# SensorsINI/v2e

Measured on NVIDIA H100. Metric: Mevents/s, higher is better.
Workload: dtype fp16 tensor-core convs (fp32 accumulate) + f64 pixel state

## Files before the change

### include/v2e_b200.h

```cpp
#ifndef V2E_B200_H
#define V2E_B200_H

#include <stdint.h>

#ifdef __cplusplus
extern "C" {
#endif

typedef enum V2eStatus {
    V2E_OK = 0,
    V2E_E_INVALID = -1,
    V2E_E_CUDA = -2,
    V2E_E_CAPACITY = -3,
    V2E_E_ITER_CAP = -4,
    V2E_E_STATE = -5,
    V2E_E_UNSUPPORTED = -6,
    V2E_E_FALLBACK = -7
} V2eStatus;

typedef enum V2eFrameDtype { V2E_U8 = 0, V2E_F32 = 1, V2E_F64 = 2 } V2eFrameDtype;

const char *v2e_last_error(void);
int v2e_version(void);
int v2e_abi_info(int *version, int *emu_cfg_size, int *frame_info_size, int *unet_weights_size);
// ... 97 lines not shown
int v2e_emu_read_counts(V2eEmu *h, int32_t *max_n, uint32_t *counts_host, int counts_cap,
                        void *stream);
int v2e_emu_phase_shot(V2eEmu *h, const void *frame_dev, int frame_dtype, double t_frame,
                       double t_previous, const float *shot_rand_dev, uint64_t capacity,
                       void *stream);
int v2e_emu_phase_emit(V2eEmu *h, double t_frame, double t_previous, float *events_out_dev,
                       uint64_t capacity, void *stream);

int v2e_emu_profile(V2eEmu *h, int enable);
int v2e_emu_profile_read4(V2eEmu *h, float *ms_sum4, int *launches4, void *stream);

int v2e_emu_state_is_f64(V2eEmu *h);
void *v2e_emu_state_ptr(V2eEmu *h, int which);

int v2e_emu_draw_noise(V2eEmu *h, uint32_t frame_index, float *leak_randn, float *shot_u01, float *pr_randn,
                       void *stream);


int v2e_conv2d_lrelu_sm100(const void *x1_dev, int C1, const void *x2_dev, int C2,
                           const void *wgt_dev, const float *bias_dev, int Cout_pad, int KH, int KW,
                           int N, int H, int W, void *out_dev, int out_cstride, int out_mode,
                           int co_real, float slope, void *stream);

int v2e_conv2d_lrelu_sm100_strip(const void *x1_dev, int C1, const void *x2_dev, int C2,
                                 const void *wgt_row_dev, const float *bias_dev, int Cout_pad, int KH,
                                 int KW, int N, int H, int W, void *out_dev, int out_cstride,
                                 int out_mode, int co_real, float slope, void *stream);
int v2e_conv_strip_pick_kc(int C1, int C2, int Cout_pad, int KH, int KW, int W);

int v2e_conv2d_up2_lrelu_sm100(const void *x_low_dev, int C, const void *wgt_fold_dev, const void *wgt_plain_dev,
                               const float *bias_dev, int Cout_pad, int N, int H_out, int W_out, void *out_dev,
                               int out_cstride, float slope, void *stream);
int v2e_conv_up2_fold_weights(const float *w_host, int cout, int cin, int Cout_pad, int C_pad, void *out_host);
int v2e_conv_up2_supported_c(int C, int Cout_pad, int W_out);

typedef struct V2eUNetWeights {
    const float *w[23];
    const float *b[23];
} V2eUNetWeights;

typedef struct V2eSlomo V2eSlomo;

int v2e_slomo_create(int H, int W, int max_batch, const V2eUNetWeights *flow,
                     const V2eUNetWeights *interp, V2eSlomo **out);
int v2e_slomo_destroy(V2eSlomo *h);
int v2e_slomo_set_pairs(V2eSlomo *h, const uint8_t *frames_u8_dev, int B, void *stream);
// ... 62 lines not shown
```

### v2e_b200/_lib.py

```python
import ctypes
import os

from . import build as _build

_LIB = None


class V2eEmuCfg(ctypes.Structure):
    _fields_ = [
        ("width", ctypes.c_int32), ("height", ctypes.c_int32),
        ("per_pixel_thres", ctypes.c_int32), ("hdr", ctypes.c_int32),
        ("pos_thres_nominal", ctypes.c_double), ("neg_thres_nominal", ctypes.c_double),
        ("cutoff_hz", ctypes.c_double), ("leak_rate_hz", ctypes.c_double),
        ("leak_jitter_fraction", ctypes.c_double), ("refractory_period_s", ctypes.c_double),
        ("shot_noise_rate_hz", ctypes.c_double), ("shot_inten_factor", ctypes.c_double),
        ("rng_mode", ctypes.c_int32), ("iter_cap", ctypes.c_int32),
        ("seed", ctypes.c_uint64),
        ("csdvs", ctypes.c_int32), ("max_frames_per_step", ctypes.c_int32),
        ("cs_tau_p_s", ctypes.c_double), ("cs_tau_h_s", ctypes.c_double),
        ("scidvs", ctypes.c_int32), ("photoreceptor_noise", ctypes.c_int32),
        ("rng_pixel_offset", ctypes.c_uint32), ("full_frame_px", ctypes.c_uint32),
        ("own_row0", ctypes.c_int32), ("own_rows", ctypes.c_int32),
        ("cs_halo_rows", ctypes.c_int32), ("reserved1", ctypes.c_int32),
    ]
# ... 39 lines not shown
    "v2e_emu_set_linlog_lut": (_i, [_vp, _vp, _vp]),
    "v2e_emu_set_fields": (_i, [_vp, _vp, _vp, _vp]),
    "v2e_emu_first_frame": (_i, [_vp, _vp, _i, _d, _d, _vp]),
    "v2e_emu_step": (_i, [_vp, _vp, _i, _i, _vp, _d, _vp, _vp, _vp, _u64, _u64, _i, _i, _vp]),
    "v2e_emu_collect": (_i, [_vp, ctypes.POINTER(V2eFrameInfo), _i, ctypes.POINTER(_i),
                             ctypes.POINTER(_u64), _vp]),
    "v2e_emu_phase_count": (_i, [_vp, _vp, _i, _d, _d, _vp, _vp, _i, _u64, _u64, _vp]),
    "v2e_emu_phase_update": (_i, [_vp, _vp, _i, _d, _d, _vp, _vp, _u64, _u64, _vp]),
    "v2e_emu_max_n_dev": (_vp, [_vp]),
    "v2e_emu_cs_begin": (_i, [_vp, _vp, _i, _d, _d, _u64, _u64, ctypes.POINTER(_i), _vp]),
    "v2e_emu_cs_pack": (_i, [_vp, _vp]),
    "v2e_emu_cs_unpack_from": (_i, [_vp, _vp, _vp, _vp]),
    "v2e_emu_cs_send_dev": (_vp, [_vp]),
    "v2e_emu_cs_chunk": (_i, [_vp, _i, _i, _vp]),
    "v2e_emu_cs_max_dev": (_vp, [_vp]),
    "v2e_emu_cs_advance": (_i, [_vp, _i, _i, _vp]),
    "v2e_emu_cs_update": (_i, [_vp, _vp, _i, _vp, _vp, _vp]),
    "v2e_emu_phase_filter": (_i, [_vp, _d, _d, _u64, _i, _vp]),
    "v2e_emu_read_counts": (_i, [_vp, ctypes.POINTER(ctypes.c_int32), _vp, _i, _vp]),
    "v2e_emu_phase_shot": (_i, [_vp, _vp, _i, _d, _d, _vp, _u64, _vp]),
    "v2e_emu_phase_emit": (_i, [_vp, _d, _d, _vp, _u64, _vp]),
    "v2e_conv2d_lrelu_sm100": (_i, [_vp, _i, _vp, _i, _vp, _vp, _i, _i, _i, _i, _i, _i, _vp, _i, _i, _i,
                                    ctypes.c_float, _vp]),
    "v2e_conv2d_lrelu_sm100_strip": (_i, [_vp, _i, _vp, _i, _vp, _vp, _i, _i, _i, _i, _i, _i, _vp, _i, _i, _i,
                                          ctypes.c_float, _vp]),
    "v2e_conv_strip_pick_kc": (_i, [_i, _i, _i, _i, _i, _i]),
    "v2e_conv2d_up2_lrelu_sm100": (_i, [_vp, _i, _vp, _vp, _vp, _i, _i, _i, _i, _vp, _i, ctypes.c_float, _vp]),
    "v2e_conv_up2_fold_weights": (_i, [_vp, _i, _i, _i, _i, _vp]),
    "v2e_conv_up2_supported_c": (_i, [_i, _i, _i]),
    "v2e_slomo_create": (_i, [_i, _i, _i, _vp, _vp, ctypes.POINTER(_vp)]),
    "v2e_slomo_destroy": (_i, [_vp]),
    "v2e_slomo_set_pairs": (_i, [_vp, _vp, _i, _vp]),
    "v2e_slomo_max_flow": (_i, [_vp, ctypes.POINTER(ctypes.c_float), _vp]),
    "v2e_slomo_interp": (_i, [_vp, _d, _vp, _vp, _vp]),
    "v2e_slomo_set_option": (_i, [_vp, _i, _i]),
    "v2e_slomo_check_finite": (_i, [_vp, ctypes.POINTER(_i), _vp]),
    "v2e_slomo_profile": (_i, [_vp, _i]),
    "v2e_slomo_profile_read": (_i, [_vp, ctypes.POINTER(ctypes.c_float), ctypes.POINTER(_i),
                                    ctypes.POINTER(ctypes.c_double), _vp]),
    "v2e_slomo_profile_read_layers": (_i, [_vp, ctypes.POINTER(ctypes.c_float), ctypes.POINTER(_i),
                                           ctypes.POINTER(ctypes.c_double), ctypes.POINTER(ctypes.c_float),
                                           ctypes.POINTER(_i), ctypes.POINTER(ctypes.c_double), _vp]),
    "v2e_slomo_flow_ptr": (_vp, [_vp]),
    "v2e_slomo_intrp_ptr": (_vp, [_vp]),
    "v2e_slomo_buffer_ptr": (_vp, [_vp, _i, _i]),
    "v2e_slomo_layer_kernel": (_i, [_vp, _i, _i]),
# ... 75 lines not shown
```

### v2e_b200/csrc/conv_tc.cu

```cuda
#include <cuda.h>
#include <cuda_fp16.h>
#include <cuda_runtime.h>
#include <stdint.h>
#include <stdio.h>
#include <string.h>
#include <vector>
#include <stdlib.h>

#include "../../include/v2e_b200.h"
#include "common.cuh"
#include "tc_common.cuh"

namespace {

constexpr int kTileH = 8, kTileW = 16, kBM = kTileH * kTileW;
constexpr int kStages = 4;
constexpr int kConvThreads = 288;
constexpr int kProducerWarp = 8;
constexpr int kConsumerWarps = 8;

struct ConvParams {
    int N, H, W;
    int C1, C2;
    int KH, KW;
    int KC;
    int BN;
    int stages;
    int co_fast;
    int tiles_x, tiles_y;
    int out_cstride;
    int out_mode;
    int co_real;
    float slope;
    const float *bias;
    void *out;
};

__device__ __forceinline__ uint8_t *align1024(uint8_t *p) { return (uint8_t *)(((uintptr_t)p + 1023) & ~(uintptr_t)1023); }

__device__ __forceinline__ float lrelu(float x, float slope) { return x > 0.f ? x : x * slope; }

template <int BN>
__device__ __forceinline__ void epilogue_row(const float (&d)[BN / 2], int i, bool inb, size_t pix, int lane,
                                             const float *bias, float slope, int out_mode, void *out, int cstride,
                                             int co0, __half2 (&h)[BN / 8]) {
#pragma unroll
    for (int j = 0; j < BN / 8; j++) {
        const int c = 8 * j + 2 * (lane & 3);
        const float x0 = lrelu(d[4 * j + 2 * i] + __ldg(bias + c), slope);
        const float x1 = lrelu(d[4 * j + 2 * i + 1] + __ldg(bias + c + 1), slope);
        h[j] = __floats2half2_rn(x0, x1);
        if (inb) {
// ... 69 lines not shown
            const uint32_t base = (uint32_t)stage * stage16;
            wgmma_fence();
            for (int j = 0; j < ksteps; j++)
                wgmma_f16<BN>(acc, desc_add(d0, base + (uint32_t)g * half16 + 2u * j), desc_add(d0, base + a16 + 2u * j),
                              (uint32_t)((it | j) != 0));
            wgmma_commit();
            wgmma_wait<1>();
            if (prev >= 0) { __syncwarp(); if (lane == 0) mbar_arrive(&empty_bar[prev]); }
            prev = stage;
            if (++stage == p.stages) { stage = 0; phase ^= 1; }
        }
        wgmma_wait<0>();
        wgmma_fence_regs(acc);
        __half2 hv[BN / 8];
#pragma unroll
        for (int i = 0; i < 2; i++) {
            const int m = 64 * g + 16 * (warp & 3) + (lane >> 2) + 8 * i;
            const int py = y0 + m / kTileW, px = x0 + m % kTileW;
            const bool inb = py < p.H && px < p.W;
            const size_t pix = ((size_t)n * p.H + py) * p.W + px;
            epilogue_row<BN>(acc, i, inb, pix, lane, p.bias + n0, p.slope, p.out_mode, p.out, p.out_cstride, n0, hv);
        }
    }
}


constexpr int kRowTile = 128;

struct StripParams {
    int N, H, W;
    int C1, C2;
    int KH, KW;
    int KC, BN;
    int tiles_x, seg_h, n_seg, n_items;
    int nslot;
    void *pool_out;
    int pool_cstride;
    int n_split, cout_pad;
    int slab_bytes;
    int w_bytes;
    int out_cstride, out_mode, co_real;
    float slope;
    const float *bias;
    void *out;
};
constexpr int kMaxSlot = 12;
// ... 379 lines not shown
extern int v2e_set_error(int code, const char *fmt, const char *detail);

typedef CUresult (*EncodeTiledFn)(CUtensorMap *, CUtensorMapDataType, cuuint32_t, void *, const cuuint64_t *,
                                  const cuuint64_t *, const cuuint32_t *, const cuuint32_t *,
                                  CUtensorMapInterleave, CUtensorMapSwizzle, CUtensorMapL2promotion,
                                  CUtensorMapFloatOOBfill);

static EncodeTiledFn encode_fn() {
    static EncodeTiledFn fn = nullptr;
    if (!fn) {
        void *p = nullptr;
        cudaDriverEntryPointQueryResult q;
        if (cudaGetDriverEntryPoint("cuTensorMapEncodeTiled", &p, cudaEnableDefault, &q) == cudaSuccess &&
            q == cudaDriverEntryPointSuccess)
            fn = (EncodeTiledFn)p;
    }
    return fn;
}

static CUtensorMapSwizzle swizzle_for(int kc) {
    return kc == 64 ? CU_TENSOR_MAP_SWIZZLE_128B : (kc == 32 ? CU_TENSOR_MAP_SWIZZLE_64B : CU_TENSOR_MAP_SWIZZLE_32B);
}

int v2e_make_act_tmap(CUtensorMap *tm, const void *ptr, int N, int H, int W, int C, int KC) {
    EncodeTiledFn fn = encode_fn();
    if (!fn) return v2e_set_error(V2E_E_CUDA, "cuTensorMapEncodeTiled unavailable%s", "");
    cuuint64_t dims[4] = {(cuuint64_t)C, (cuuint64_t)W, (cuuint64_t)H, (cuuint64_t)N};
    cuuint64_t strides[3] = {(cuuint64_t)C * 2, (cuuint64_t)W * C * 2, (cuuint64_t)H * W * C * 2};
    cuuint32_t box[4] = {(cuuint32_t)KC, (cuuint32_t)kTileW, (cuuint32_t)kTileH, 1};
    cuuint32_t es[4] = {1, 1, 1, 1};
    CUresult r = fn(tm, CU_TENSOR_MAP_DATA_TYPE_FLOAT16, 4, (void *)ptr, dims, strides, box, es,
                    CU_TENSOR_MAP_INTERLEAVE_NONE, swizzle_for(KC), CU_TENSOR_MAP_L2_PROMOTION_L2_256B,
                    CU_TENSOR_MAP_FLOAT_OOB_FILL_NONE);
    if (r != CUDA_SUCCESS) {
        snprintf(g_conv_err, sizeof(g_conv_err), "activation map N=%d H=%d W=%d C=%d KC=%d CUresult=%d", N, H, W, C, KC, (int)r);
        return v2e_set_error(V2E_E_CUDA, "cuTensorMapEncodeTiled failed: %s", g_conv_err);
    }
    return V2E_OK;
}

int v2e_make_wgt_tmap(CUtensorMap *tm, const void *ptr, int Cout_pad, int Ktot, int KC, int BN) {
    EncodeTiledFn fn = encode_fn();
    if (!fn) return v2e_set_error(V2E_E_CUDA, "cuTensorMapEncodeTiled unavailable%s", "");
    cuuint64_t dims[2] = {(cuuint64_t)Ktot, (cuuint64_t)Cout_pad};
    cuuint64_t strides[1] = {(cuuint64_t)Ktot * 2};
    cuuint32_t box[2] = {(cuuint32_t)KC, (cuuint32_t)BN};
    cuuint32_t es[2] = {1, 1};
    CUresult r = fn(tm, CU_TENSOR_MAP_DATA_TYPE_FLOAT16, 2, (void *)ptr, dims, strides, box, es,
                    CU_TENSOR_MAP_INTERLEAVE_NONE, swizzle_for(KC), CU_TENSOR_MAP_L2_PROMOTION_L2_256B,
                    CU_TENSOR_MAP_FLOAT_OOB_FILL_NONE);
    if (r != CUDA_SUCCESS) {
        snprintf(g_conv_err, sizeof(g_conv_err), "weight map Cout=%d K=%d KC=%d BN=%d CUresult=%d", Cout_pad, Ktot, KC, BN, (int)r);
        return v2e_set_error(V2E_E_CUDA, "cuTensorMapEncodeTiled failed: %s", g_conv_err);
    }
    return V2E_OK;
}

int v2e_conv_pick_kc(int C1, int C2) {
    int g = C2 ? (C1 < C2 ? C1 : C2) : C1;
    return g % 64 == 0 ? 64 : (g % 32 == 0 ? 32 : 16);
}
int v2e_conv_pick_bn(int Cout_pad) { return Cout_pad >= 128 ? 128 : Cout_pad; }

struct V2eConvLaunch {
    CUtensorMap tmA, tmA2, tmB;
    ConvParams p;
    dim3 grid;
    size_t smem;
};

int v2e_conv_prepare(V2eConvLaunch *L, const void *x1, int C1, const void *x2, int C2, const void *wgt,
                     const float *bias, int Cout_pad, int KH, int KW, int N, int H, int W, void *out,
                     int out_cstride, int out_mode, int co_real, float slope) {
    if (C1 % 16 || C2 % 16 || !(Cout_pad == 16 || Cout_pad == 32 || Cout_pad == 64 || (Cout_pad > 0 && Cout_pad % 128 == 0)))
        return v2e_set_error(V2E_E_INVALID, "conv: channel counts must be padded to 16 (Cout to 16/32/64/128k)%s", "");
    memset(L, 0, sizeof(*L));
    ConvParams &p = L->p;
    p.N = N; p.H = H; p.W = W; p.C1 = C1; p.C2 = C2; p.KH = KH; p.KW = KW;
    p.KC = v2e_conv_pick_kc(C1, C2);
    p.BN = v2e_conv_pick_bn(Cout_pad);
    p.stages = kStages;
    p.tiles_x = (W + kTileW - 1) / kTileW;
    p.tiles_y = (H + kTileH - 1) / kTileH;
    p.out_cstride = out_cstride; p.out_mode = out_mode; p.co_real = co_real; p.slope = slope;
    p.bias = bias; p.out = out;
    int rc;
    if ((rc = v2e_make_act_tmap(&L->tmA, x1, N, H, W, C1, p.KC))) return rc;
    if (C2) { if ((rc = v2e_make_act_tmap(&L->tmA2, x2, N, H, W, C2, p.KC))) return rc; }
    else L->tmA2 = L->tmA;
    if ((rc = v2e_make_wgt_tmap(&L->tmB, wgt, Cout_pad, KH * KW * (C1 + C2), p.KC, p.BN))) return rc;
    {
        static int co_fast = -1;
        if (co_fast < 0) { const char *e = getenv("V2E_CONV_CO_FAST"); co_fast = e ? atoi(e) : 1; }
        const unsigned tiles = (unsigned)(p.tiles_x * p.tiles_y * N), cob = (unsigned)(Cout_pad / p.BN);
        p.co_fast = (co_fast && cob > 1 && tiles <= 65535u) ? 1 : 0;
        L->grid = p.co_fast ? dim3(cob, tiles, 1) : dim3(tiles, cob, 1);
    }
    size_t stage = (size_t)kBM * p.KC * 2 + (((size_t)p.BN * p.KC * 2 + 1023) & ~(size_t)1023);
    L->smem = stage * p.stages + 1024;
    return V2E_OK;
}

template <int BN>
static cudaError_t conv_launch_bn(const V2eConvLaunch *L, cudaStream_t st) {
    static PerDeviceOnce attr_once;
    if (attr_once.first()) cudaFuncSetAttribute(conv_tc_kernel<BN>, cudaFuncAttributeMaxDynamicSharedMemorySize, 200 * 1024);
    conv_tc_kernel<BN><<<L->grid, kConvThreads, L->smem, st>>>(L->tmA, L->tmA2, L->tmB, L->p);
    return cudaGetLastError();
}

int v2e_conv_launch(const V2eConvLaunch *L, cudaStream_t st) {
    cudaError_t e;
    switch (L->p.BN) {
        case 16: e = conv_launch_bn<16>(L, st); break;
        case 32: e = conv_launch_bn<32>(L, st); break;
        case 64: e = conv_launch_bn<64>(L, st); break;
        case 128: e = conv_launch_bn<128>(L, st); break;
        default: return v2e_set_error(V2E_E_UNSUPPORTED, "conv_tc_kernel: unsupported tile width%s", "");
    }
    if (e != cudaSuccess) return v2e_set_error(V2E_E_CUDA, "conv_tc_kernel launch: %s", cudaGetErrorString(e));
    return V2E_OK;
}

size_t v2e_conv_launch_size(void) { return sizeof(V2eConvLaunch); }

extern "C" int v2e_conv2d_lrelu_sm100(const void *x1_dev, int C1, const void *x2_dev, int C2,
                                      const void *wgt_dev, const float *bias_dev, int Cout_pad, int KH, int KW,
                                      int N, int H, int W, void *out_dev, int out_cstride, int out_mode,
                                      int co_real, float slope, void *stream) {
    V2eConvLaunch L;
    int rc = v2e_conv_prepare(&L, x1_dev, C1, x2_dev, C2, wgt_dev, bias_dev, Cout_pad, KH, KW, N, H, W, out_dev,
                              out_cstride, out_mode, co_real, slope);
    if (rc) return rc;
    return v2e_conv_launch(&L, (cudaStream_t)stream);
}

struct V2eStripLaunch {
    CUtensorMap tmA, tmA2, tmB;
    StripParams p;
    int grid;
    size_t smem;
};

static int make_rowseg_tmap(CUtensorMap *tm, const void *ptr, int N, int H, int W, int C, int KC, int KW) {
    EncodeTiledFn fn = encode_fn();
    if (!fn) return v2e_set_error(V2E_E_CUDA, "cuTensorMapEncodeTiled unavailable%s", "");
    cuuint64_t dims[4] = {(cuuint64_t)C, (cuuint64_t)W, (cuuint64_t)H, (cuuint64_t)N};
    cuuint64_t strides[3] = {(cuuint64_t)C * 2, (cuuint64_t)W * C * 2, (cuuint64_t)H * W * C * 2};
    cuuint32_t box[4] = {(cuuint32_t)KC, (cuuint32_t)(kRowTile + KW - 1), 1, 1};
    cuuint32_t es[4] = {1, 1, 1, 1};
    CUresult r = fn(tm, CU_TENSOR_MAP_DATA_TYPE_FLOAT16, 4, (void *)ptr, dims, strides, box, es,
                    CU_TENSOR_MAP_INTERLEAVE_NONE, swizzle_for(KC), CU_TENSOR_MAP_L2_PROMOTION_L2_256B,
                    CU_TENSOR_MAP_FLOAT_OOB_FILL_NONE);
    if (r != CUDA_SUCCESS) return v2e_set_error(V2E_E_CUDA, "cuTensorMapEncodeTiled failed for a strip row map%s", "");
    return V2E_OK;
}

// ... 305 lines not shown
```

### v2e_b200/csrc/slomo.cu

```cuda
#include <cuda.h>
#include <cuda_fp16.h>
#include <cuda_runtime.h>
#include <math.h>
#include <stdint.h>
#include <stdio.h>
#include <string.h>
#include <stdlib.h>

#include <vector>

#include "../../include/v2e_b200.h"
#include "common.cuh"

struct V2eConvLaunch;
int v2e_conv_prepare(V2eConvLaunch *L, const void *x1, int C1, const void *x2, int C2, const void *wgt,
                     const float *bias, int Cout_pad, int KH, int KW, int N, int H, int W, void *out,
                     int out_cstride, int out_mode, int co_real, float slope);
int v2e_conv_launch(const V2eConvLaunch *L, cudaStream_t st);
size_t v2e_conv_launch_size(void);
struct V2eStripLaunch;
int v2e_strip_pick(int C1, int C2, int Cout_pad, int KH, int KW, int W, int *nslot_out);
size_t v2e_strip_launch_size(void);
int v2e_strip_pool_supported(int C1, int C2, int Cout_pad, int KH, int KW, int H, int W);
int v2e_strip_prepare(V2eStripLaunch *L, const void *x1, int C1, const void *x2, int C2, const void *wgt_row,
                      const float *bias, int Cout_pad, int KH, int KW, int N, int H, int W, void *out,
                      int out_cstride, int out_mode, int co_real, float slope, int n_sms, void *pool_out,
                      int pool_cstride);
int v2e_strip_launch(const V2eStripLaunch *L, cudaStream_t st);
struct V2eUpLaunch;
int v2e_conv_up2_supported(int C, int Cout_pad, int W_out);
extern "C" int v2e_conv_up2_fold_weights(const float *w, int cout, int cin, int Cout_pad, int C_pad, void *out_host);
size_t v2e_conv_up2_launch_size(void);
int v2e_conv_up2_prepare(V2eUpLaunch *L, const void *x_low, int C, const void *wgt_fold, const void *wgt_plain,
                         const float *bias, int Cout_pad, int N, int H, int W, void *out, int out_cstride, float slope,
                         int n_sms);
int v2e_conv_up2_launch(const V2eUpLaunch *L, cudaStream_t st);
int v2e_set_error(int code, const char *fmt, const char *detail);

#define CU(call)                                                                              \
    do {                                                                                      \
// ... 410 lines not shown
    for (int l = 0; l < 5; l++) {
        cudaFree(h->pool[l]); cudaFree(h->da[l]); cudaFree(h->s[l]);
        cudaFree(h->up[l]); cudaFree(h->ua[l]); cudaFree(h->ub[l]);
    }
    for (cudaEvent_t e : h->ev) cudaEventDestroy(e);
    delete h;
    return V2E_OK;
}

static int conv(V2eSlomo *h, const UNet &u, int li, const __half *x1, const __half *x2, int B, int H, int W, void *out,
                int out_mode, cudaStream_t st, __half *pool_out = nullptr) {
    int rc;
    const bool row = u.row_kc[li] != 0 && !h->force_tap_kernel;
    V2eConvLaunch *L = (V2eConvLaunch *)h->launch_mem.data();
    V2eStripLaunch *R = (V2eStripLaunch *)h->row_mem.data();
    h->ran[&u == &h->interp][li] = row ? (pool_out ? V2E_SLOMO_KERNEL_STRIP_POOL : V2E_SLOMO_KERNEL_STRIP)
                                       : V2E_SLOMO_KERNEL_TAP;
    if (row)
        rc = v2e_strip_prepare(R, x1, u.c1p[li], x2, x2 ? u.c2p[li] : 0, u.w_row[li], u.b[li], u.cout_pad[li], u.L[li].k,
                               u.L[li].k, B, H, W, out, u.cout_pad[li], out_mode, u.L[li].cout, kSlope, h->n_sms,
                               pool_out, u.cout_pad[li]);
    else
        rc = v2e_conv_prepare(L, x1, u.c1p[li], x2, x2 ? u.c2p[li] : 0, u.w[li], u.b[li], u.cout_pad[li], u.L[li].k,
                              u.L[li].k, B, H, W, out, u.cout_pad[li], out_mode, u.L[li].cout, kSlope);
    if (rc) return rc;
    if (h->profile) {
        if (h->ev_used + 2 > h->ev.size()) {
            size_t old = h->ev.size();
            h->ev.resize(old + 512);
            for (size_t i = old; i < h->ev.size(); i++) cudaEventCreate(&h->ev[i]);
        }
        cudaEventRecord(h->ev[h->ev_used], st);
    }
    rc = row ? v2e_strip_launch(R, st) : v2e_conv_launch(L, st);
    if (h->profile) {
        cudaEventRecord(h->ev[h->ev_used + 1], st);
        h->ev_used += 2;
        const LayerSpec &l = u.L[li];
        const double fl = 2.0 * B * H * W * (double)l.cout * (l.cin1 + l.cin2) * l.k * l.k;
        h->conv_flops += fl;
        h->ev_layer.push_back(li);
        h->ev_flops.push_back(fl);
    }
    return rc;
}

static int conv_up2(V2eSlomo *h, const UNet &u, int li, const __half *x_low, int B, int H, int W, void *out, cudaStream_t st) {
// ... 273 lines not shown
```

### v2e_b200/csrc/tc_common.cuh

```cuda
#pragma once
#include <cuda.h>
#include <cuda_runtime.h>
#include <stdint.h>

__device__ __forceinline__ uint32_t smem_u32(const void *p) { return (uint32_t)__cvta_generic_to_shared(p); }

__device__ __forceinline__ void mbar_init(uint64_t *bar, uint32_t count) {
    asm volatile("mbarrier.init.shared::cta.b64 [%0], %1;" ::"r"(smem_u32(bar)), "r"(count) : "memory");
}
__device__ __forceinline__ void fence_barrier_init() { asm volatile("fence.mbarrier_init.release.cluster;" ::: "memory"); }
__device__ __forceinline__ void mbar_expect_tx(uint64_t *bar, uint32_t bytes) {
    asm volatile("mbarrier.arrive.expect_tx.shared::cta.b64 _, [%0], %1;" ::"r"(smem_u32(bar)), "r"(bytes) : "memory");
}
__device__ __forceinline__ void mbar_arrive(uint64_t *bar) {
    asm volatile("mbarrier.arrive.shared::cta.b64 _, [%0];" ::"r"(smem_u32(bar)) : "memory");
}
__device__ __forceinline__ void mbar_wait(uint64_t *bar, uint32_t parity) {
    const uint32_t addr = smem_u32(bar);
    uint32_t done;
    do {
        asm volatile(
            "{\n\t.reg .pred p;\n\t"
            "mbarrier.try_wait.parity.shared::cta.b64 p, [%1], %2;\n\t"
            "selp.u32 %0, 1, 0, p;\n\t}"
            : "=r"(done) : "r"(addr), "r"(parity) : "memory");
    } while (!done);
}

__device__ __forceinline__ void prefetch_tmap(const CUtensorMap *tm) {
    asm volatile("prefetch.tensormap [%0];" ::"l"((uint64_t)tm) : "memory");
}
__device__ __forceinline__ void tma_load_4d(void *dst, const CUtensorMap *tm, uint64_t *bar, int c0, int c1, int c2, int c3) {
    asm volatile(
        "cp.async.bulk.tensor.4d.shared::cluster.global.tile.mbarrier::complete_tx::bytes [%0], [%1, {%3, %4, %5, %6}], [%2];"
        ::"r"(smem_u32(dst)), "l"((uint64_t)tm), "r"(smem_u32(bar)), "r"(c0), "r"(c1), "r"(c2), "r"(c3) : "memory");
}
__device__ __forceinline__ void tma_load_2d(void *dst, const CUtensorMap *tm, uint64_t *bar, int c0, int c1) {
    asm volatile(
        "cp.async.bulk.tensor.2d.shared::cluster.global.tile.mbarrier::complete_tx::bytes [%0], [%1, {%3, %4}], [%2];"
        ::"r"(smem_u32(dst)), "l"((uint64_t)tm), "r"(smem_u32(bar)), "r"(c0), "r"(c1) : "memory");
}

__device__ __forceinline__ uint32_t elect_one() {
    uint32_t pred;
    asm volatile("{\n\t.reg .pred p;\n\telect.sync _|p, 0xffffffff;\n\tselp.u32 %0, 1, 0, p;\n\t}" : "=r"(pred));
    return pred;
}

__device__ __forceinline__ void wgmma_fence() { asm volatile("wgmma.fence.sync.aligned;" ::: "memory"); }
__device__ __forceinline__ void wgmma_commit() { asm volatile("wgmma.commit_group.sync.aligned;" ::: "memory"); }
template <int N>
__device__ __forceinline__ void wgmma_wait() { asm volatile("wgmma.wait_group.sync.aligned %0;" ::"n"(N) : "memory"); }
template <int R>
__device__ __forceinline__ void wgmma_fence_regs(float (&d)[R]) {
#pragma unroll
    for (int i = 0; i < R; i++) asm volatile("" : "+f"(d[i])::"memory");
}

__device__ __forceinline__ void wgmma_m64n16k16(float (&d)[8], uint64_t adesc, uint64_t bdesc, uint32_t scale_d) {
    asm volatile(
        "{\n\t.reg .pred p;\n\tsetp.ne.b32 p, %10, 0;\n\t"
        "wgmma.mma_async.sync.aligned.m64n16k16.f32.f16.f16 {%0, %1, %2, %3, %4, %5, %6, %7}, %8, %9, p, 1, 1, 0, 0;\n\t}"
        : "+f"(d[0]), "+f"(d[1]), "+f"(d[2]), "+f"(d[3]), "+f"(d[4]), "+f"(d[5]), "+f"(d[6]), "+f"(d[7])
        : "l"(adesc), "l"(bdesc), "r"(scale_d) : "memory");
}
__device__ __forceinline__ void wgmma_m64n32k16(float (&d)[16], uint64_t adesc, uint64_t bdesc, uint32_t scale_d) {
    asm volatile(
        "{\n\t.reg .pred p;\n\tsetp.ne.b32 p, %18, 0;\n\t"
        "wgmma.mma_async.sync.aligned.m64n32k16.f32.f16.f16 {%0, %1, %2, %3, %4, %5, %6, %7, %8, %9, %10, %11, %12, %13, %14, %15}, %16, %17, p, 1, 1, 0, 0;\n\t}"
        : "+f"(d[0]), "+f"(d[1]), "+f"(d[2]), "+f"(d[3]), "+f"(d[4]), "+f"(d[5]), "+f"(d[6]), "+f"(d[7]), "+f"(d[8]), "+f"(d[9]), "+f"(d[10]), "+f"(d[11]), "+f"(d[12]), "+f"(d[13]), "+f"(d[14]), "+f"(d[15])
        : "l"(adesc), "l"(bdesc), "r"(scale_d) : "memory");
}
__device__ __forceinline__ void wgmma_m64n64k16(float (&d)[32], uint64_t adesc, uint64_t bdesc, uint32_t scale_d) {
    asm volatile(
        "{\n\t.reg .pred p;\n\tsetp.ne.b32 p, %34, 0;\n\t"
        "wgmma.mma_async.sync.aligned.m64n64k16.f32.f16.f16 {%0, %1, %2, %3, %4, %5, %6, %7, %8, %9, %10, %11, %12, %13, %14, %15, %16, %17, %18, %19, %20, %21, %22, %23, %24, %25, %26, %27, %28, %29, %30, %31}, %32, %33, p, 1, 1, 0, 0;\n\t}"
        : "+f"(d[0]), "+f"(d[1]), "+f"(d[2]), "+f"(d[3]), "+f"(d[4]), "+f"(d[5]), "+f"(d[6]), "+f"(d[7]), "+f"(d[8]), "+f"(d[9]), "+f"(d[10]), "+f"(d[11]), "+f"(d[12]), "+f"(d[13]), "+f"(d[14]), "+f"(d[15]), "+f"(d[16]), "+f"(d[17]), "+f"(d[18]), "+f"(d[19]), "+f"(d[20]), "+f"(d[21]), "+f"(d[22]), "+f"(d[23]), "+f"(d[24]), "+f"(d[25]), "+f"(d[26]), "+f"(d[27]), "+f"(d[28]), "+f"(d[29]), "+f"(d[30]), "+f"(d[31])
        : "l"(adesc), "l"(bdesc), "r"(scale_d) : "memory");
}
__device__ __forceinline__ void wgmma_m64n128k16(float (&d)[64], uint64_t adesc, uint64_t bdesc, uint32_t scale_d) {
    asm volatile(
        "{\n\t.reg .pred p;\n\tsetp.ne.b32 p, %66, 0;\n\t"
        "wgmma.mma_async.sync.aligned.m64n128k16.f32.f16.f16 {%0, %1, %2, %3, %4, %5, %6, %7, %8, %9, %10, %11, %12, %13, %14, %15, %16, %17, %18, %19, %20, %21, %22, %23, %24, %25, %26, %27, %28, %29, %30, %31, %32, %33, %34, %35, %36, %37, %38, %39, %40, %41, %42, %43, %44, %45, %46, %47, %48, %49, %50, %51, %52, %53, %54, %55, %56, %57, %58, %59, %60, %61, %62, %63}, %64, %65, p, 1, 1, 0, 0;\n\t}"
        : "+f"(d[0]), "+f"(d[1]), "+f"(d[2]), "+f"(d[3]), "+f"(d[4]), "+f"(d[5]), "+f"(d[6]), "+f"(d[7]), "+f"(d[8]), "+f"(d[9]), "+f"(d[10]), "+f"(d[11]), "+f"(d[12]), "+f"(d[13]), "+f"(d[14]), "+f"(d[15]), "+f"(d[16]), "+f"(d[17]), "+f"(d[18]), "+f"(d[19]), "+f"(d[20]), "+f"(d[21]), "+f"(d[22]), "+f"(d[23]), "+f"(d[24]), "+f"(d[25]), "+f"(d[26]), "+f"(d[27]), "+f"(d[28]), "+f"(d[29]), "+f"(d[30]), "+f"(d[31]), "+f"(d[32]), "+f"(d[33]), "+f"(d[34]), "+f"(d[35]), "+f"(d[36]), "+f"(d[37]), "+f"(d[38]), "+f"(d[39]), "+f"(d[40]), "+f"(d[41]), "+f"(d[42]), "+f"(d[43]), "+f"(d[44]), "+f"(d[45]), "+f"(d[46]), "+f"(d[47]), "+f"(d[48]), "+f"(d[49]), "+f"(d[50]), "+f"(d[51]), "+f"(d[52]), "+f"(d[53]), "+f"(d[54]), "+f"(d[55]), "+f"(d[56]), "+f"(d[57]), "+f"(d[58]), "+f"(d[59]), "+f"(d[60]), "+f"(d[61]), "+f"(d[62]), "+f"(d[63])
        : "l"(adesc), "l"(bdesc), "r"(scale_d) : "memory");
}
template <int N>
__device__ __forceinline__ void wgmma_f16(float (&d)[N / 2], uint64_t adesc, uint64_t bdesc, uint32_t scale_d) {
    if constexpr (N == 16) wgmma_m64n16k16(d, adesc, bdesc, scale_d);
    else if constexpr (N == 32) wgmma_m64n32k16(d, adesc, bdesc, scale_d);
    else if constexpr (N == 64) wgmma_m64n64k16(d, adesc, bdesc, scale_d);
    else wgmma_m64n128k16(d, adesc, bdesc, scale_d);
}

__device__ __forceinline__ uint32_t swizzle_layout(int kc) { return kc == 64 ? 1u : (kc == 32 ? 2u : 3u); }
__device__ __forceinline__ uint64_t make_smem_desc(uint32_t smem_addr, uint32_t layout_type, uint32_t sbo_bytes) {
    uint64_t d = 0;
    d |= (uint64_t)((smem_addr & 0x3FFFFu) >> 4);
    d |= (uint64_t)1 << 16;
    d |= (uint64_t)((sbo_bytes >> 4) & 0x3FFFu) << 32;
    d |= (uint64_t)layout_type << 62;
    return d;
}
__device__ __forceinline__ uint64_t desc_add(uint64_t d, uint32_t add16) { return d + (uint64_t)add16; }
```

Measured before the change: 50.58.

## Add wide 256x128 and 128x256 conv tiles with cost-model tile selection

Adds a new warp-specialized conv kernel that computes larger CTA tiles (two M halves per warpgroup, or N=256 via m64n256 wgmma), so each loaded operand slab is reused across more output. A simple cost model picks legacy or wide tiles per layer from the wave count and a bytes-versus-flops estimate, and it is applied by default in the SloMo UNet path. An optional cluster-multicast mode for weight tiles is available through an environment variable. The wide tiles double the accumulator registers and enlarge stages, which can lower occupancy, and they can leave SMs idle through wave quantization on small layers.

```diff
diff --git a/include/v2e_b200.h b/include/v2e_b200.h
--- a/include/v2e_b200.h
+++ b/include/v2e_b200.h
@@ -143,6 +143,18 @@
                            int N, int H, int W, void *out_dev, int out_cstride, int out_mode,
                            int co_real, float slope, void *stream);
 
+enum {
+    V2E_CONV_TILE_AUTO = -1,
+    V2E_CONV_TILE_LEGACY = 0,
+    V2E_CONV_TILE_256x128 = 1,
+    V2E_CONV_TILE_128x256 = 2
+};
+int v2e_conv2d_lrelu_sm100_tile(const void *x1_dev, int C1, const void *x2_dev, int C2,
+                                const void *wgt_dev, const float *bias_dev, int Cout_pad, int KH, int KW,
+                                int N, int H, int W, void *out_dev, int out_cstride, int out_mode,
+                                int co_real, float slope, int tile, int multicast, void *stream);
+int v2e_conv_pick_tile(int C1, int C2, int Cout_pad, int KH, int KW, int N, int H, int W, int n_sms);
+
 int v2e_conv2d_lrelu_sm100_strip(const void *x1_dev, int C1, const void *x2_dev, int C2,
                                  const void *wgt_row_dev, const float *bias_dev, int Cout_pad, int KH,
                                  int KW, int N, int H, int W, void *out_dev, int out_cstride,
diff --git a/v2e_b200/_lib.py b/v2e_b200/_lib.py
--- a/v2e_b200/_lib.py
+++ b/v2e_b200/_lib.py
@@ -85,6 +85,9 @@
     "v2e_emu_phase_emit": (_i, [_vp, _d, _d, _vp, _u64, _vp]),
     "v2e_conv2d_lrelu_sm100": (_i, [_vp, _i, _vp, _i, _vp, _vp, _i, _i, _i, _i, _i, _i, _vp, _i, _i, _i,
                                     ctypes.c_float, _vp]),
+    "v2e_conv2d_lrelu_sm100_tile": (_i, [_vp, _i, _vp, _i, _vp, _vp, _i, _i, _i, _i, _i, _i, _vp, _i, _i, _i,
+                                         ctypes.c_float, _i, _i, _vp]),
+    "v2e_conv_pick_tile": (_i, [_i, _i, _i, _i, _i, _i, _i, _i, _i]),
     "v2e_conv2d_lrelu_sm100_strip": (_i, [_vp, _i, _vp, _i, _vp, _vp, _i, _i, _i, _i, _i, _i, _vp, _i, _i, _i,
                                           ctypes.c_float, _vp]),
     "v2e_conv_strip_pick_kc": (_i, [_i, _i, _i, _i, _i, _i]),
diff --git a/v2e_b200/csrc/conv_tc.cu b/v2e_b200/csrc/conv_tc.cu
--- a/v2e_b200/csrc/conv_tc.cu
+++ b/v2e_b200/csrc/conv_tc.cu
@@ -1,6 +1,7 @@
 #include <cuda.h>
 #include <cuda_fp16.h>
 #include <cuda_runtime.h>
+#include <math.h>
 #include <stdint.h>
 #include <stdio.h>
 #include <string.h>
@@ -28,6 +29,7 @@
     int stages;
     int co_fast;
     int tiles_x, tiles_y;
+    int n_tiles;
     int out_cstride;
     int out_mode;
     int co_real;
@@ -143,6 +145,137 @@
             epilogue_row<BN>(acc, i, inb, pix, lane, p.bias + n0, p.slope, p.out_mode, p.out, p.out_cstride, n0, hv);
         }
     }
+}
+
+template <int MH, int BN, bool MC>
+__global__ void __launch_bounds__(kConvThreads, 1)
+conv_wide_kernel(const __grid_constant__ CUtensorMap tmA, const __grid_constant__ CUtensorMap tmA2,
+                 const __grid_constant__ CUtensorMap tmB, const ConvParams p) {
+    constexpr int TH = kTileH * MH, BM = kBM * MH;
+    extern __shared__ __align__(1024) uint8_t smem_raw[];
+    uint8_t *smem = align1024(smem_raw);
+    const uint32_t a_bytes = BM * p.KC * 2;
+    const uint32_t b_bytes = BN * p.KC * 2;
+    const uint32_t stage_bytes = a_bytes + b_bytes;
+    __shared__ __align__(8) uint64_t full_bar[kStages], empty_bar[kStages];
+
+    const int warp = threadIdx.x >> 5, lane = threadIdx.x & 31;
+    const int tile_g = p.co_fast ? blockIdx.y : blockIdx.x;
+    const bool live = tile_g < p.n_tiles;
+    const int tile = live ? tile_g : p.n_tiles - 1;
+    const int tx = tile % p.tiles_x, ty = (tile / p.tiles_x) % p.tiles_y, n = tile / (p.tiles_x * p.tiles_y);
+    const int x0 = tx * kTileW, y0 = ty * TH;
+    const int n0 = (p.co_fast ? blockIdx.x : blockIdx.y) * BN;
+    const int Ctot = p.C1 + p.C2;
+    const int slabs = Ctot / p.KC;
+    const int k_iters = p.KH * p.KW * slabs;
+    const uint32_t crank = MC ? cluster_ctarank() : 0u;
+
+    if (threadIdx.x == 0) {
+        for (int s = 0; s < kStages; s++) {
+            mbar_init(&full_bar[s], 1);
+            mbar_init(&empty_bar[s], (MC ? 2 : 1) * kConsumerWarps);
+        }
+        fence_barrier_init();
+    }
+    if (warp == kProducerWarp && lane == 0) {
+        prefetch_tmap(&tmA);
+        if (p.C2) prefetch_tmap(&tmA2);
+        prefetch_tmap(&tmB);
+    }
+    if constexpr (MC) cluster_sync();
+    else __syncthreads();
+
+    if (warp == kProducerWarp) {
+        if (lane == 0) {
+            int stage = 0;
+            uint32_t phase = 0;
+            const int ph = p.KH / 2, pw = p.KW / 2;
+            for (int tap = 0; tap < p.KH * p.KW; tap++) {
+                const int r = tap / p.KW, s = tap % p.KW;
+                for (int sl = 0; sl < slabs; sl++) {
+                    mbar_wait(&empty_bar[stage], phase ^ 1);
+                    uint8_t *sa = smem + stage * stage_bytes, *sb = sa + a_bytes;
+                    mbar_expect_tx(&full_bar[stage], a_bytes + b_bytes);
+                    const int c = sl * p.KC;
+                    if (c < p.C1) tma_load_4d(sa, &tmA, &full_bar[stage], c, x0 + s - pw, y0 + r - ph, n);
+                    else tma_load_4d(sa, &tmA2, &full_bar[stage], c - p.C1, x0 + s - pw, y0 + r - ph, n);
+                    if constexpr (MC)
+                        tma_load_2d_multicast(sb + crank * (b_bytes / 2), &tmB, &full_bar[stage], tap * Ctot + c,
+                                              n0 + (int)crank * (BN / 2), (uint16_t)0x3);
+                    else
+                        tma_load_2d(sb, &tmB, &full_bar[stage], tap * Ctot + c, n0);
+                    if (++stage == p.stages) { stage = 0; phase ^= 1; }
+                }
+            }
+        }
+    } else {
+        const int g = __shfl_sync(0xffffffffu, warp >> 2, 0);
+        const uint64_t d0 = make_smem_desc(smem_u32(smem), swizzle_layout(p.KC), 8u * p.KC * 2u);
+        const uint32_t stage16 = stage_bytes >> 4, a16 = a_bytes >> 4, q16 = (64u * p.KC * 2u) >> 4;
+        const int ksteps = p.KC / 16;
+        float acc[MH][BN / 2];
+#pragma unroll
+        for (int h = 0; h < MH; h++) {
+#pragma unroll
+            for (int i = 0; i < BN / 2; i++) acc[h][i] = 0.f;
+            wgmma_fence_regs(acc[h]);
+        }
+        int stage = 0, prev = -1;
+        uint32_t phase = 0;
+        for (int it = 0; it < k_iters; it++) {
+            mbar_wait(&full_bar[stage], phase);
+            const uint32_t base = (uint32_t)stage * stage16;
+            wgmma_fence();
+            for (int j = 0; j < ksteps; j++) {
+#pragma unroll
+                for (int h = 0; h < MH; h++)
+                    wgmma_f16<BN>(acc[h], desc_add(d0, base + (uint32_t)(g * MH + h) * q16 + 2u * j),
+                                  desc_add(d0, base + a16 + 2u * j), (uint32_t)((it | j) != 0));
+            }
+            wgmma_commit();
+            wgmma_wait<1>();
+            if (prev >= 0) {
+                __syncwarp();
+                if (lane == 0) {
+                    mbar_arrive(&empty_bar[prev]);
+                    if constexpr (MC) mbar_arrive_cluster(&empty_bar[prev], crank ^ 1u);
+                }
+            }
+            prev = stage;
+            if (++stage == p.stages) { stage = 0; phase ^= 1; }
+        }
+        wgmma_wait<0>();
+#pragma unroll
+        for (int h = 0; h < MH; h++) wgmma_fence_regs(acc[h]);
+        if (live) {
+            const float *bias = p.bias + n0;
+            __half *out = (__half *)p.out + n0;
+#pragma unroll
+            for (int h = 0; h < MH; h++) {
+                size_t pix[2];
+                bool inb[2];
+#pragma unroll
+                for (int i = 0; i < 2; i++) {
+                    const int m = 64 * (g * MH + h) + 16 * (warp & 3) + (lane >> 2) + 8 * i;
+                    const int py = y0 + m / kTileW, px = x0 + m % kTileW;
+                    inb[i] = py < p.H && px < p.W;
+                    pix[i] = (((size_t)n * p.H + py) * p.W + px) * p.out_cstride;
+                }
+#pragma unroll
+                for (int j = 0; j < BN / 8; j++) {
+                    const int c = 8 * j + 2 * (lane & 3);
+                    const float2 b = __ldg((const float2 *)(bias + c));
+#pragma unroll
+                    for (int i = 0; i < 2; i++)
+                        if (inb[i])
+                            *(__half2 *)(out + pix[i] + c) = __floats2half2_rn(lrelu(acc[h][4 * j + 2 * i] + b.x, p.slope),
+                                                                               lrelu(acc[h][4 * j + 2 * i + 1] + b.y, p.slope));
+                }
+            }
+        }
+    }
+    if constexpr (MC) cluster_sync();
 }
 
 
@@ -568,12 +701,12 @@
     return kc == 64 ? CU_TENSOR_MAP_SWIZZLE_128B : (kc == 32 ? CU_TENSOR_MAP_SWIZZLE_64B : CU_TENSOR_MAP_SWIZZLE_32B);
 }
 
-int v2e_make_act_tmap(CUtensorMap *tm, const void *ptr, int N, int H, int W, int C, int KC) {
+static int make_act_tmap_h(CUtensorMap *tm, const void *ptr, int N, int H, int W, int C, int KC, int tile_h) {
     EncodeTiledFn fn = encode_fn();
     if (!fn) return v2e_set_error(V2E_E_CUDA, "cuTensorMapEncodeTiled unavailable%s", "");
     cuuint64_t dims[4] = {(cuuint64_t)C, (cuuint64_t)W, (cuuint64_t)H, (cuuint64_t)N};
     cuuint64_t strides[3] = {(cuuint64_t)C * 2, (cuuint64_t)W * C * 2, (cuuint64_t)H * W * C * 2};
-    cuuint32_t box[4] = {(cuuint32_t)KC, (cuuint32_t)kTileW, (cuuint32_t)kTileH, 1};
+    cuuint32_t box[4] = {(cuuint32_t)KC, (cuuint32_t)kTileW, (cuuint32_t)tile_h, 1};
     cuuint32_t es[4] = {1, 1, 1, 1};
     CUresult r = fn(tm, CU_TENSOR_MAP_DATA_TYPE_FLOAT16, 4, (void *)ptr, dims, strides, box, es,
                     CU_TENSOR_MAP_INTERLEAVE_NONE, swizzle_for(KC), CU_TENSOR_MAP_L2_PROMOTION_L2_256B,
@@ -583,6 +716,9 @@
         return v2e_set_error(V2E_E_CUDA, "cuTensorMapEncodeTiled failed: %s", g_conv_err);
     }
     return V2E_OK;
+}
+int v2e_make_act_tmap(CUtensorMap *tm, const void *ptr, int N, int H, int W, int C, int KC) {
+    return make_act_tmap_h(tm, ptr, N, H, W, C, KC, kTileH);
 }
 
 int v2e_make_wgt_tmap(CUtensorMap *tm, const void *ptr, int Cout_pad, int Ktot, int KC, int BN) {
@@ -608,41 +744,95 @@
 }
 int v2e_conv_pick_bn(int Cout_pad) { return Cout_pad >= 128 ? 128 : Cout_pad; }
 
+static void tile_shape(int tile, int Cout_pad, int *mh, int *bn) {
+    *mh = tile == V2E_CONV_TILE_256x128 ? 2 : 1;
+    *bn = tile == V2E_CONV_TILE_128x256 ? 256 : (tile == V2E_CONV_TILE_256x128 ? 128 : v2e_conv_pick_bn(Cout_pad));
+}
+
+extern "C" int v2e_conv_pick_tile(int C1, int C2, int Cout_pad, int KH, int KW, int N, int H, int W, int n_sms) {
+    (void)KH; (void)KW;
+    const int kc = v2e_conv_pick_kc(C1, C2);
+    if (n_sms < 1) n_sms = 1;
+    int best = V2E_CONV_TILE_LEGACY;
+    double best_cost = 0.0;
+    for (int tile = V2E_CONV_TILE_LEGACY; tile <= V2E_CONV_TILE_128x256; tile++) {
+        int mh, bn;
+        tile_shape(tile, Cout_pad, &mh, &bn);
+        const bool wide = tile != V2E_CONV_TILE_LEGACY;
+        if (wide && (kc != 64 || Cout_pad % bn || (tile == V2E_CONV_TILE_256x128) != (Cout_pad == 128))) continue;
+        long tiles = (long)((W + kTileW - 1) / kTileW) * ((H + kTileH * mh - 1) / (kTileH * mh)) * N;
+        const long ctas = tiles * (Cout_pad / bn);
+        const long waves = (ctas + n_sms - 1) / n_sms;
+        const double a_bytes = (double)kBM * mh * kc * 2, b_bytes = (double)bn * kc * 2;
+        const double flops = 2.0 * kBM * mh * bn * kc;
+        const double per_stage = fmax((a_bytes + b_bytes) / 24.0, flops / 4096.0);
+        const double cost = (double)waves * per_stage;
+        if (tile == V2E_CONV_TILE_LEGACY || cost < best_cost) { best = tile; best_cost = cost; }
+    }
+    return best;
+}
+
 struct V2eConvLaunch {
     CUtensorMap tmA, tmA2, tmB;
     ConvParams p;
-    dim3 grid;
+    dim3 grid, cluster;
+    int mh, multicast;
     size_t smem;
 };
 
+static int conv_tile_env() {
+    static int v = -1;
+    if (v < 0) {
+        const char *e = getenv("V2E_CONV_TILE");
+        v = !e ? 0 : (!strcmp(e, "legacy") ? 1 : (!strcmp(e, "multicast") ? 2 : 0));
+    }
+    return v;
+}
+
 int v2e_conv_prepare(V2eConvLaunch *L, const void *x1, int C1, const void *x2, int C2, const void *wgt,
                      const float *bias, int Cout_pad, int KH, int KW, int N, int H, int W, void *out,
-                     int out_cstride, int out_mode, int co_real, float slope) {
+                     int out_cstride, int out_mode, int co_real, float slope, int tile, int multicast, int n_sms) {
     if (C1 % 16 || C2 % 16 || !(Cout_pad == 16 || Cout_pad == 32 || Cout_pad == 64 || (Cout_pad > 0 && Cout_pad % 128 == 0)))
         return v2e_set_error(V2E_E_INVALID, "conv: channel counts must be padded to 16 (Cout to 16/32/64/128k)%s", "");
+    if (tile == V2E_CONV_TILE_AUTO) {
+        const int env = conv_tile_env();
+        tile = env == 1 ? V2E_CONV_TILE_LEGACY : v2e_conv_pick_tile(C1, C2, Cout_pad, KH, KW, N, H, W, n_sms);
+        multicast = env == 2;
+    }
+    if (tile < V2E_CONV_TILE_LEGACY || tile > V2E_CONV_TILE_128x256)
+        return v2e_set_error(V2E_E_INVALID, "conv: unknown tile%s", "");
     memset(L, 0, sizeof(*L));
     ConvParams &p = L->p;
+    int mh, bn;
+    tile_shape(tile, Cout_pad, &mh, &bn);
+    const bool wide = tile != V2E_CONV_TILE_LEGACY;
     p.N = N; p.H = H; p.W = W; p.C1 = C1; p.C2 = C2; p.KH = KH; p.KW = KW;
     p.KC = v2e_conv_pick_kc(C1, C2);
-    p.BN = v2e_conv_pick_bn(Cout_pad);
+    p.BN = bn;
+    if (wide && (Cout_pad % bn || out_mode != 0))
+        return v2e_set_error(V2E_E_INVALID, "conv: the wide tiles need fp16 output and Cout_pad a multiple of their width%s", "");
     p.stages = kStages;
     p.tiles_x = (W + kTileW - 1) / kTileW;
-    p.tiles_y = (H + kTileH - 1) / kTileH;
+    p.tiles_y = (H + kTileH * mh - 1) / (kTileH * mh);
+    p.n_tiles = p.tiles_x * p.tiles_y * N;
     p.out_cstride = out_cstride; p.out_mode = out_mode; p.co_real = co_real; p.slope = slope;
     p.bias = bias; p.out = out;
+    L->mh = mh;
+    L->multicast = wide && multicast;
     int rc;
-    if ((rc = v2e_make_act_tmap(&L->tmA, x1, N, H, W, C1, p.KC))) return rc;
-    if (C2) { if ((rc = v2e_make_act_tmap(&L->tmA2, x2, N, H, W, C2, p.KC))) return rc; }
+    if ((rc = make_act_tmap_h(&L->tmA, x1, N, H, W, C1, p.KC, kTileH * mh))) return rc;
+    if (C2) { if ((rc = make_act_tmap_h(&L->tmA2, x2, N, H, W, C2, p.KC, kTileH * mh))) return rc; }
     else L->tmA2 = L->tmA;
-    if ((rc = v2e_make_wgt_tmap(&L->tmB, wgt, Cout_pad, KH * KW * (C1 + C2), p.KC, p.BN))) return rc;
+    if ((rc = v2e_make_wgt_tmap(&L->tmB, wgt, Cout_pad, KH * KW * (C1 + C2), p.KC, L->multicast ? bn / 2 : bn))) return rc;
     {
         static int co_fast = -1;
         if (co_fast < 0) { const char *e = getenv("V2E_CONV_CO_FAST"); co_fast = e ? atoi(e) : 1; }
-        const unsigned tiles = (unsigned)(p.tiles_x * p.tiles_y * N), cob = (unsigned)(Cout_pad / p.BN);
+        const unsigned tiles = (unsigned)(L->multicast ? (p.n_tiles + 1) & ~1 : p.n_tiles), cob = (unsigned)(Cout_pad / p.BN);
         p.co_fast = (co_fast && cob > 1 && tiles <= 65535u) ? 1 : 0;
         L->grid = p.co_fast ? dim3(cob, tiles, 1) : dim3(tiles, cob, 1);
-    }
-    size_t stage = (size_t)kBM * p.KC * 2 + (((size_t)p.BN * p.KC * 2 + 1023) & ~(size_t)1023);
+        L->cluster = !L->multicast ? dim3(1, 1, 1) : (p.co_fast ? dim3(1, 2, 1) : dim3(2, 1, 1));
+    }
+    size_t stage = (size_t)kBM * mh * p.KC * 2 + (((size_t)p.BN * p.KC * 2 + 1023) & ~(size_t)1023);
     L->smem = stage * p.stages + 1024;
     return V2E_OK;
 }
@@ -655,9 +845,31 @@
     return cudaGetLastError();
 }
 
+template <int MH, int BN, bool MC>
+static cudaError_t conv_launch_wide(const V2eConvLaunch *L, cudaStream_t st) {
+    static PerDeviceOnce attr_once;
+    if (attr_once.first())
+        cudaFuncSetAttribute(conv_wide_kernel<MH, BN, MC>, cudaFuncAttributeMaxDynamicSharedMemorySize, 226 * 1024);
+    cudaLaunchConfig_t cfg = {};
+    cfg.gridDim = L->grid;
+    cfg.blockDim = dim3(kConvThreads, 1, 1);
+    cfg.dynamicSmemBytes = L->smem;
+    cfg.stream = st;
+    cudaLaunchAttribute attr[1];
+    attr[0].id = cudaLaunchAttributeClusterDimension;
+    attr[0].val.clusterDim.x = L->cluster.x;
+    attr[0].val.clusterDim.y = L->cluster.y;
+    attr[0].val.clusterDim.z = 1;
+    cfg.attrs = attr;
+    cfg.numAttrs = 1;
+    return cudaLaunchKernelEx(&cfg, conv_wide_kernel<MH, BN, MC>, L->tmA, L->tmA2, L->tmB, L->p);
+}
+
 int v2e_conv_launch(const V2eConvLaunch *L, cudaStream_t st) {
     cudaError_t e;
-    switch (L->p.BN) {
+    if (L->mh == 2 && L->p.BN == 128) e = L->multicast ? conv_launch_wide<2, 128, true>(L, st) : conv_launch_wide<2, 128, false>(L, st);
+    else if (L->mh == 1 && L->p.BN == 256) e = L->multicast ? conv_launch_wide<1, 256, true>(L, st) : conv_launch_wide<1, 256, false>(L, st);
+    else switch (L->p.BN) {
         case 16: e = conv_launch_bn<16>(L, st); break;
         case 32: e = conv_launch_bn<32>(L, st); break;
         case 64: e = conv_launch_bn<64>(L, st); break;
@@ -670,15 +882,30 @@
 
 size_t v2e_conv_launch_size(void) { return sizeof(V2eConvLaunch); }
 
+static int device_sms() {
+    int dev = 0, sms = 132;
+    cudaGetDevice(&dev);
+    cudaDeviceGetAttribute(&sms, cudaDevAttrMultiProcessorCount, dev);
+    return sms;
+}
+
+extern "C" int v2e_conv2d_lrelu_sm100_tile(const void *x1_dev, int C1, const void *x2_dev, int C2,
+                                           const void *wgt_dev, const float *bias_dev, int Cout_pad, int KH, int KW,
+                                           int N, int H, int W, void *out_dev, int out_cstride, int out_mode,
+                                           int co_real, float slope, int tile, int multicast, void *stream) {
+    V2eConvLaunch L;
+    int rc = v2e_conv_prepare(&L, x1_dev, C1, x2_dev, C2, wgt_dev, bias_dev, Cout_pad, KH, KW, N, H, W, out_dev,
+                              out_cstride, out_mode, co_real, slope, tile, multicast, device_sms());
+    if (rc) return rc;
+    return v2e_conv_launch(&L, (cudaStream_t)stream);
+}
+
 extern "C" int v2e_conv2d_lrelu_sm100(const void *x1_dev, int C1, const void *x2_dev, int C2,
                                       const void *wgt_dev, const float *bias_dev, int Cout_pad, int KH, int KW,
                                       int N, int H, int W, void *out_dev, int out_cstride, int out_mode,
                                       int co_real, float slope, void *stream) {
-    V2eConvLaunch L;
-    int rc = v2e_conv_prepare(&L, x1_dev, C1, x2_dev, C2, wgt_dev, bias_dev, Cout_pad, KH, KW, N, H, W, out_dev,
-                              out_cstride, out_mode, co_real, slope);
-    if (rc) return rc;
-    return v2e_conv_launch(&L, (cudaStream_t)stream);
+    return v2e_conv2d_lrelu_sm100_tile(x1_dev, C1, x2_dev, C2, wgt_dev, bias_dev, Cout_pad, KH, KW, N, H, W, out_dev,
+                                       out_cstride, out_mode, co_real, slope, V2E_CONV_TILE_AUTO, 0, stream);
 }
 
 struct V2eStripLaunch {
diff --git a/v2e_b200/csrc/slomo.cu b/v2e_b200/csrc/slomo.cu
--- a/v2e_b200/csrc/slomo.cu
+++ b/v2e_b200/csrc/slomo.cu
@@ -15,7 +15,7 @@
 struct V2eConvLaunch;
 int v2e_conv_prepare(V2eConvLaunch *L, const void *x1, int C1, const void *x2, int C2, const void *wgt,
                      const float *bias, int Cout_pad, int KH, int KW, int N, int H, int W, void *out,
-                     int out_cstride, int out_mode, int co_real, float slope);
+                     int out_cstride, int out_mode, int co_real, float slope, int tile, int multicast, int n_sms);
 int v2e_conv_launch(const V2eConvLaunch *L, cudaStream_t st);
 size_t v2e_conv_launch_size(void);
 struct V2eStripLaunch;
@@ -472,7 +472,8 @@
                                pool_out, u.cout_pad[li]);
     else
         rc = v2e_conv_prepare(L, x1, u.c1p[li], x2, x2 ? u.c2p[li] : 0, u.w[li], u.b[li], u.cout_pad[li], u.L[li].k,
-                              u.L[li].k, B, H, W, out, u.cout_pad[li], out_mode, u.L[li].cout, kSlope);
+                              u.L[li].k, B, H, W, out, u.cout_pad[li], out_mode, u.L[li].cout, kSlope,
+                              V2E_CONV_TILE_AUTO, 0, h->n_sms);
     if (rc) return rc;
     if (h->profile) {
         if (h->ev_used + 2 > h->ev.size()) {
diff --git a/v2e_b200/csrc/tc_common.cuh b/v2e_b200/csrc/tc_common.cuh
--- a/v2e_b200/csrc/tc_common.cuh
+++ b/v2e_b200/csrc/tc_common.cuh
@@ -39,6 +39,28 @@
     asm volatile(
         "cp.async.bulk.tensor.2d.shared::cluster.global.tile.mbarrier::complete_tx::bytes [%0], [%1, {%3, %4}], [%2];"
         ::"r"(smem_u32(dst)), "l"((uint64_t)tm), "r"(smem_u32(bar)), "r"(c0), "r"(c1) : "memory");
+}
+
+__device__ __forceinline__ uint32_t cluster_ctarank() {
+    uint32_t r;
+    asm volatile("mov.u32 %0, %%cluster_ctarank;" : "=r"(r));
+    return r;
+}
+__device__ __forceinline__ void cluster_sync() {
+    asm volatile("barrier.cluster.arrive.release;\n\tbarrier.cluster.wait.acquire;" ::: "memory");
+}
+__device__ __forceinline__ void mbar_arrive_cluster(uint64_t *bar, uint32_t cta) {
+    asm volatile(
+        "{\n\t.reg .b32 ra;\n\tmapa.shared::cluster.u32 ra, %0, %1;\n\t"
+        "mbarrier.arrive.release.cluster.shared::cluster.b64 _, [ra];\n\t}"
+        ::"r"(smem_u32(bar)), "r"(cta) : "memory");
+}
+__device__ __forceinline__ void tma_load_2d_multicast(void *dst, const CUtensorMap *tm, uint64_t *bar, int c0, int c1,
+                                                      uint16_t mask) {
+    asm volatile(
+        "cp.async.bulk.tensor.2d.shared::cluster.global.tile.mbarrier::complete_tx::bytes.multicast::cluster"
+        " [%0], [%1, {%3, %4}], [%2], %5;"
+        ::"r"(smem_u32(dst)), "l"((uint64_t)tm), "r"(smem_u32(bar)), "r"(c0), "r"(c1), "h"(mask) : "memory");
 }
 
 __device__ __forceinline__ uint32_t elect_one() {
@@ -85,12 +107,20 @@
         : "+f"(d[0]), "+f"(d[1]), "+f"(d[2]), "+f"(d[3]), "+f"(d[4]), "+f"(d[5]), "+f"(d[6]), "+f"(d[7]), "+f"(d[8]), "+f"(d[9]), "+f"(d[10]), "+f"(d[11]), "+f"(d[12]), "+f"(d[13]), "+f"(d[14]), "+f"(d[15]), "+f"(d[16]), "+f"(d[17]), "+f"(d[18]), "+f"(d[19]), "+f"(d[20]), "+f"(d[21]), "+f"(d[22]), "+f"(d[23]), "+f"(d[24]), "+f"(d[25]), "+f"(d[26]), "+f"(d[27]), "+f"(d[28]), "+f"(d[29]), "+f"(d[30]), "+f"(d[31]), "+f"(d[32]), "+f"(d[33]), "+f"(d[34]), "+f"(d[35]), "+f"(d[36]), "+f"(d[37]), "+f"(d[38]), "+f"(d[39]), "+f"(d[40]), "+f"(d[41]), "+f"(d[42]), "+f"(d[43]), "+f"(d[44]), "+f"(d[45]), "+f"(d[46]), "+f"(d[47]), "+f"(d[48]), "+f"(d[49]), "+f"(d[50]), "+f"(d[51]), "+f"(d[52]), "+f"(d[53]), "+f"(d[54]), "+f"(d[55]), "+f"(d[56]), "+f"(d[57]), "+f"(d[58]), "+f"(d[59]), "+f"(d[60]), "+f"(d[61]), "+f"(d[62]), "+f"(d[63])
         : "l"(adesc), "l"(bdesc), "r"(scale_d) : "memory");
 }
+__device__ __forceinline__ void wgmma_m64n256k16(float (&d)[128], uint64_t adesc, uint64_t bdesc, uint32_t scale_d) {
+    asm volatile(
+        "{\n\t.reg .pred p;\n\tsetp.ne.b32 p, %130, 0;\n\t"
+        "wgmma.mma_async.sync.aligned.m64n256k16.f32.f16.f16 {%0, %1, %2, %3, %4, %5, %6, %7, %8, %9, %10, %11, %12, %13, %14, %15, %16, %17, %18, %19, %20, %21, %22, %23, %24, %25, %26, %27, %28, %29, %30, %31, %32, %33, %34, %35, %36, %37, %38, %39, %40, %41, %42, %43, %44, %45, %46, %47, %48, %49, %50, %51, %52, %53, %54, %55, %56, %57, %58, %59, %60, %61, %62, %63, %64, %65, %66, %67, %68, %69, %70, %71, %72, %73, %74, %75, %76, %77, %78, %79, %80, %81, %82, %83, %84, %85, %86, %87, %88, %89, %90, %91, %92, %93, %94, %95, %96, %97, %98, %99, %100, %101, %102, %103, %104, %105, %106, %107, %108, %109, %110, %111, %112, %113, %114, %115, %116, %117, %118, %119, %120, %121, %122, %123, %124, %125, %126, %127}, %128, %129, p, 1, 1, 0, 0;\n\t}"
+        : "+f"(d[0]), "+f"(d[1]), "+f"(d[2]), "+f"(d[3]), "+f"(d[4]), "+f"(d[5]), "+f"(d[6]), "+f"(d[7]), "+f"(d[8]), "+f"(d[9]), "+f"(d[10]), "+f"(d[11]), "+f"(d[12]), "+f"(d[13]), "+f"(d[14]), "+f"(d[15]), "+f"(d[16]), "+f"(d[17]), "+f"(d[18]), "+f"(d[19]), "+f"(d[20]), "+f"(d[21]), "+f"(d[22]), "+f"(d[23]), "+f"(d[24]), "+f"(d[25]), "+f"(d[26]), "+f"(d[27]), "+f"(d[28]), "+f"(d[29]), "+f"(d[30]), "+f"(d[31]), "+f"(d[32]), "+f"(d[33]), "+f"(d[34]), "+f"(d[35]), "+f"(d[36]), "+f"(d[37]), "+f"(d[38]), "+f"(d[39]), "+f"(d[40]), "+f"(d[41]), "+f"(d[42]), "+f"(d[43]), "+f"(d[44]), "+f"(d[45]), "+f"(d[46]), "+f"(d[47]), "+f"(d[48]), "+f"(d[49]), "+f"(d[50]), "+f"(d[51]), "+f"(d[52]), "+f"(d[53]), "+f"(d[54]), "+f"(d[55]), "+f"(d[56]), "+f"(d[57]), "+f"(d[58]), "+f"(d[59]), "+f"(d[60]), "+f"(d[61]), "+f"(d[62]), "+f"(d[63]), "+f"(d[64]), "+f"(d[65]), "+f"(d[66]), "+f"(d[67]), "+f"(d[68]), "+f"(d[69]), "+f"(d[70]), "+f"(d[71]), "+f"(d[72]), "+f"(d[73]), "+f"(d[74]), "+f"(d[75]), "+f"(d[76]), "+f"(d[77]), "+f"(d[78]), "+f"(d[79]), "+f"(d[80]), "+f"(d[81]), "+f"(d[82]), "+f"(d[83]), "+f"(d[84]), "+f"(d[85]), "+f"(d[86]), "+f"(d[87]), "+f"(d[88]), "+f"(d[89]), "+f"(d[90]), "+f"(d[91]), "+f"(d[92]), "+f"(d[93]), "+f"(d[94]), "+f"(d[95]), "+f"(d[96]), "+f"(d[97]), "+f"(d[98]), "+f"(d[99]), "+f"(d[100]), "+f"(d[101]), "+f"(d[102]), "+f"(d[103]), "+f"(d[104]), "+f"(d[105]), "+f"(d[106]), "+f"(d[107]), "+f"(d[108]), "+f"(d[109]), "+f"(d[110]), "+f"(d[111]), "+f"(d[112]), "+f"(d[113]), "+f"(d[114]), "+f"(d[115]), "+f"(d[116]), "+f"(d[117]), "+f"(d[118]), "+f"(d[119]), "+f"(d[120]), "+f"(d[121]), "+f"(d[122]), "+f"(d[123]), "+f"(d[124]), "+f"(d[125]), "+f"(d[126]), "+f"(d[127])
+        : "l"(adesc), "l"(bdesc), "r"(scale_d) : "memory");
+}
 template <int N>
 __device__ __forceinline__ void wgmma_f16(float (&d)[N / 2], uint64_t adesc, uint64_t bdesc, uint32_t scale_d) {
     if constexpr (N == 16) wgmma_m64n16k16(d, adesc, bdesc, scale_d);
     else if constexpr (N == 32) wgmma_m64n32k16(d, adesc, bdesc, scale_d);
     else if constexpr (N == 64) wgmma_m64n64k16(d, adesc, bdesc, scale_d);
-    else wgmma_m64n128k16(d, adesc, bdesc, scale_d);
+    else if constexpr (N == 128) wgmma_m64n128k16(d, adesc, bdesc, scale_d);
+    else wgmma_m64n256k16(d, adesc, bdesc, scale_d);
 }
 
 __device__ __forceinline__ uint32_t swizzle_layout(int kc) { return kc == 64 ? 1u : (kc == 32 ? 2u : 3u); }
```

After: 55.19, median of 6. 1.09x the previous value.
